# Cryptum169/another-cuda-sift

Hardware: AMD Instinct MI355X
Metric: detectAndCompute Mpix/s + 2kx2k 128-D match ms at 1/2/4/8 MI355X (higher is better)
Workload: dtype f32; 1 GPU; C2: detectAndCompute on 1920x1200 frames, 16 per step per GPU (one launch per stage for the batch), numOctaveLayers=3 (5 DoG scales/octave), numOctaves=3, upscale=false, numFeatures=5000; frames HBM-resident; frames_per_launch=16, streams_per_gpu=2, parallelism=frame-sharded x1, no data-path collective, descriptor_mode=fixed-point (default), keypoints_per_frame=4366

## Files before the change

### another-cuda-sift_amd/csrc/pyramid.hip

```cpp
#include <array>
#include <cstring>
#include <utility>

#include "sift_kernels.h"
#include "sift_math.h"

namespace sift_amd {

__device__ __forceinline__ void up_coeff(int d, int slen, int& s, float& a0, float& a1) {
    float f = (float)d * 0.5f - 0.25f;
    int si = (int)floorf(f);
    f -= (float)si;
    if (si < 0) { f = 0.f; si = 0; }
    if (si >= slen - 1) { f = 0.f; si = slen - 1; }
    s = si;
    a0 = 1.f - f;
    a1 = f;
}

__device__ __forceinline__ float dpp_left_or(float own, float v) {
    return __int_as_float(__builtin_amdgcn_update_dpp(__float_as_int(own), __float_as_int(v), 0x138, 0xf, 0xf, false));
}
__device__ __forceinline__ float dpp_right_or(float own, float v) {
    return __int_as_float(__builtin_amdgcn_update_dpp(__float_as_int(own), __float_as_int(v), 0x130, 0xf, 0xf, false));
}

template <typename T>
__global__ __launch_bounds__(256) void k_upsample2x(const T* __restrict__ src, int spitch, int W, int H,
                                                    float* __restrict__ dst, int dpitch, long sfs, long dfs) {
    src = fptr(src, blockIdx.z * sfs);
    dst = fptr(dst, blockIdx.z * dfs);
    const int per = (H + 4 * (int)gridDim.y - 1) / (4 * (int)gridDim.y);
    const int m0 = (blockIdx.y * 4 + (threadIdx.x >> 6)) * per;
    if (m0 >= H) return;
    const int mEnd = min(m0 + per, H);
    const int lane = threadIdx.x & 63, base = blockIdx.x * 256;
    const int c[2] = {base + 2 * lane, base + 128 + 2 * lane};
    const int xe = lane == 0 ? max(base - 1, 0) : min(base + 256, W - 1);
    const bool vec = sizeof(T) == 4 && (reinterpret_cast<uintptr_t>(src) & 7) == 0 && (spitch & 1) == 0;
    struct Raw {
        float v[2][2], e;
    };
    auto load = [&](int y, Raw& r) {
        const T* row = src + (size_t)min(max(y, 0), H - 1) * spitch;
#pragma unroll
        for (int h = 0; h < 2; h++) {
            if (vec && c[h] + 1 < W) {
                const float2 q = *reinterpret_cast<const float2*>(row + c[h]);
                r.v[h][0] = q.x;
                r.v[h][1] = q.y;
            } else {
                r.v[h][0] = (float)row[min(c[h], W - 1)];
                r.v[h][1] = (float)row[min(c[h] + 1, W - 1)];
            }
        }
        r.e = (float)row[xe];
    };
    auto horiz = [&](const Raw& r, float (&hh)[8]) {
        float w[2][4];
        const float a1_63 = __int_as_float(__builtin_amdgcn_readlane(__float_as_int(r.v[0][1]), 63));
        const float b0_0 = __int_as_float(__builtin_amdgcn_readlane(__float_as_int(r.v[1][0]), 0));
        w[0][0] = dpp_left_or(r.e, r.v[0][1]);
        w[0][3] = dpp_right_or(b0_0, r.v[0][0]);
        w[1][0] = dpp_left_or(a1_63, r.v[1][1]);
        w[1][3] = dpp_right_or(r.e, r.v[1][0]);
#pragma unroll
        for (int h = 0; h < 2; h++) {
            w[h][1] = r.v[h][0];
            w[h][2] = r.v[h][1];
            if (c[h] >= 1 && c[h] + 2 < W) {
                hh[4 * h] = w[h][0] * 0.25f + w[h][1] * 0.75f;
                hh[4 * h + 1] = w[h][1] * 0.75f + w[h][2] * 0.25f;
                hh[4 * h + 2] = w[h][1] * 0.25f + w[h][2] * 0.75f;
                hh[4 * h + 3] = w[h][2] * 0.75f + w[h][3] * 0.25f;
            } else {
#pragma unroll
                for (int t = 0; t < 4; t++) {
                    int sx;
                    float ax0, ax1;
                    up_coeff(min(2 * c[h] + t, 2 * W - 1), W, sx, ax0, ax1);
                    const int k0 = min(max(sx - c[h] + 1, 0), 3), k1 = min(max(min(sx + 1, W - 1) - c[h] + 1, 0), 3);
                    const float s0 = k0 == 0 ? w[h][0] : (k0 == 1 ? w[h][1] : (k0 == 2 ? w[h][2] : w[h][3]));
                    const float s1 = k1 == 0 ? w[h][0] : (k1 == 1 ? w[h][1] : (k1 == 2 ? w[h][2] : w[h][3]));
                    hh[4 * h + t] = s0 * ax0 + s1 * ax1;
                }
            }
        }
    };
    Raw rr;
    float hp[8], hc[8], hn[8];
    load(m0 - 1, rr);
    horiz(rr, hp);
    load(m0, rr);
    horiz(rr, hc);
    load(m0 + 1, rr);
    for (int m = m0; m < mEnd; m++) {
        horiz(rr, hn);
        if (m + 1 < mEnd) load(m + 2, rr);
#pragma unroll
        for (int v = 0; v < 2; v++) {
            int sy;
            float ay0, ay1;
            up_coeff(2 * m + v, H, sy, ay0, ay1);
            const bool r0c = sy == m, r1c = min(sy + 1, H - 1) == m;
            float o[8];
#pragma unroll
            for (int i = 0; i < 8; i++) o[i] = (r0c ? hc[i] : hp[i]) * ay0 + (r1c ? hc[i] : hn[i]) * ay1;
            float* d = dst + (size_t)(2 * m + v) * dpitch;
#pragma unroll
            for (int h = 0; h < 2; h++) {
                if (c[h] + 2 <= W) {
                    *reinterpret_cast<float4*>(d + 2 * c[h]) = make_float4(o[4 * h], o[4 * h + 1], o[4 * h + 2], o[4 * h + 3]);
                } else if (c[h] < W) {
                    d[2 * c[h]] = o[4 * h];
                    d[2 * c[h] + 1] = o[4 * h + 1];
                }
            }
        }
#pragma unroll
        for (int i = 0; i < 8; i++) {
            hp[i] = hc[i];
            hc[i] = hn[i];
        }
    }
}

dim3 up_grid(int W, int H, int nf) {
    const int per = nf > 1 ? 8 : 2;
    return dim3((W + 255) / 256, (H + 4 * per - 1) / (4 * per), nf);
}

void launch_upsample2x(const float* src, int spitch, int W, int H, float* dst, int dpitch, const Frames& fr, long sfs,
                       hipStream_t s) {
    hipLaunchKernelGGL(k_upsample2x<float>, up_grid(W, H, fr.nf), dim3(256), 0, s, src, spitch, W, H, dst, dpitch, sfs,
                       fr.stride);
}

void launch_upsample2x_u8(const uint8_t* src, int spitch, int W, int H, float* dst, int dpitch, const Frames& fr,
                          long sfs, hipStream_t s) {
    hipLaunchKernelGGL(k_upsample2x<uint8_t>, up_grid(W, H, fr.nf), dim3(256), 0, s, src, spitch, W, H, dst, dpitch, sfs, fr.stride);
}

typedef float f32x4 __attribute__((ext_vector_type(4)));
typedef float f32x2 __attribute__((ext_vector_type(2)));

__device__ __forceinline__ f32x2 pk_mov_hi_lo(f32x2 a, f32x2 b) {
    f32x2 r;
    __asm__("v_pk_mov_b32 %0, %1, %2 op_sel:[1,0]" : "=v"(r) : "v"(a), "v"(b));
    return r;
}
constexpr int BLUR_TW = 64;
constexpr int BLUR_TH = 64;
constexpr int kBlurBigTiles = 2048;
static_assert(BLUR_TH % 32 == 0, "blur tile height: 8-row column blocks for 4 or 8 waves");
static int blur_waves(int tiles) { return tiles >= kBlurBigTiles ? 4 : 8; }

struct BlurJob {
    const void* src;
    float* dst;
    DecOut dec;
    unsigned* range_keys;
    Counters* zero_ctr;
    int spitch, W, H, dpitch, tilesX, ntiles;
    int nf;
    long sfs, dfs;
    Taps taps;
};

constexpr bool kBlurIW16 = true;
constexpr bool kBlurX4Ld = true;
constexpr bool kBlurX4LdBig = true;
constexpr int kBlurX4LdMaxR = 24;
constexpr bool kBlurX4St = true;
constexpr bool kBlurDma = true;
template <int R>
constexpr int blur_org() {
    return kBlurX4Ld && R <= 8 ? 8 : kBlurX4Ld && kBlurX4LdBig && R <= kBlurX4LdMaxR ? (R + 3) & ~3 : R;
}
constexpr bool kBlurIW112 = false;
template <int R>
constexpr int blur_iw() {
    return kBlurIW16 && R <= 8 ? ((BLUR_TW + 2 * blur_org<R>() + 15) / 32) * 32 + 16
           : kBlurIW112 && R >= 11 && R <= 24 ? 112
                                                   : (BLUR_TW + 2 * blur_org<R>() + 3) & ~3;
}
template <int R>
constexpr int blur_lds_floats() {
    return blur_iw<R>() * (BLUR_TH + 2 * R) + 4;
}


template <int R, typename T, int NWAVES>
__device__ __forceinline__ void blur_tile(const BlurJob& J, int blk, float* __restrict__ in) {
    constexpr int BLUR_NW = NWAVES;
    constexpr int BLUR_CB = BLUR_TH / (8 * BLUR_NW);
    constexpr int IW = blur_iw<R>();
    constexpr int IH = BLUR_TH + 2 * R;
    constexpr int ORG = blur_org<R>();
    constexpr int SA = (ORG - R) & ~3, SS = (ORG - R) & 3;
    constexpr int NW = (SS + 2 * R + 4 + 3) / 4;
    static_assert(BLUR_TW - 4 + SA + 4 * NW <= IW, "row window inside the LDS row");
    const int t = xcd_tile(blk, J.ntiles * J.nf);
    const int f = t / J.ntiles, tile = t - f * J.ntiles;
    const T* __restrict__ src = fptr(static_cast<const T*>(J.src), f * J.sfs);
    float* __restrict__ dst = fptr(J.dst, f * J.dfs);
    float* __restrict__ dec_out = J.dec.p ? fptr(J.dec.p, f * J.dfs) : nullptr;
    unsigned* __restrict__ range_keys = J.range_keys ? fptr(J.range_keys, f * J.dfs) : nullptr;
    Counters* __restrict__ zero_ctr = J.zero_ctr ? fptr(J.zero_ctr, f * J.dfs) : nullptr;
    const int spitch = J.spitch, W = J.W, H = J.H, dpitch = J.dpitch;
    const Taps& taps = J.taps;
    float* const mid = in;
    const int x0 = (tile % J.tilesX) * BLUR_TW, y0 = (tile / J.tilesX) * BLUR_TH;
    const int tid = threadIdx.x, lane = tid & 63, wave = tid >> 6;
    if (zero_ctr && tile == 0 && tid < (int)(sizeof(Counters) / 4))
        reinterpret_cast<unsigned*>(zero_ctr)[tid] =
            tid == offsetof(Counters, pad[1]) / 4 ? zero_ctr->pad[1] & ~((1u << kHostReqShift) - 1) : 0u;

    {
        constexpr int RW = BLUR_TW + 2 * R;
        constexpr int RPW = (IH + BLUR_NW - 1) / BLUR_NW;
        const int wv = __builtin_amdgcn_readfirstlane(wave);
        const bool single = W > R + 1 && H > R + 1;
        auto refl = [&](int p, int len) {
            if (single) {
                p = p < 0 ? -p : (p >= len ? 2 * len - 2 - p : p);
                return min(max(p, 0), len - 1);
            }
            return reflect101(p, len);
        };
        const int gx0 = refl(x0 - R + lane, W), gx1 = refl(x0 - R + 64 + min(lane, RW - 65), W);
        constexpr int ES = (int)sizeof(T);
        const __amdgpu_buffer_rsrc_t rsrc = __builtin_amdgcn_make_buffer_rsrc(
            const_cast<T*>(src), 0, (int)min((long)spitch * H * ES, 0x7fffffffL), 0x00020000);
        const unsigned c0 = (unsigned)gx0 * ES, c1 = (unsigned)gx1 * ES;
        const int rowB = spitch * ES;
        float v0[RPW], v1[RPW];
        auto ld = [&](int i, int roff) {
            if constexpr (ES == 1) {
                v0[i] = (float)__builtin_amdgcn_raw_buffer_load_b8(rsrc, c0, roff, 0);
                v1[i] = (float)__builtin_amdgcn_raw_buffer_load_b8(rsrc, c1, roff, 0);
            } else {
                v0[i] = __builtin_bit_cast(float, __builtin_amdgcn_raw_buffer_load_b32(rsrc, c0, roff, 0));
                v1[i] = __builtin_bit_cast(float, __builtin_amdgcn_raw_buffer_load_b32(rsrc, c1, roff, 0));
            }
        };
        constexpr int QW = (BLUR_TW + 2 * ORG) / 4;
        const bool x4 = ES == 4 && ORG % 4 == 0 && ORG >= R && x0 >= ORG &&
                        x0 + BLUR_TW + ORG <= W && y0 - R >= 0 && y0 - R + IH <= H;
        if (x4) {
            static_assert(!(ES == 4 && ORG % 4 == 0) || 4 * QW <= IW, "x4 staging row inside the LDS row");
            constexpr int NQ = QW * IH, NT = 64 * BLUR_NW, QPT = (NQ + NT - 1) / NT;
            const int rb0 = (y0 - R) * spitch + x0 - ORG;
            if constexpr (kBlurDma && IW == 4 * QW) {
                const float* fsrc = reinterpret_cast<const float*>(src);
#pragma unroll
                for (int u = 0; u < QPT; u++) {
                    const int idx = tid + NT * u;
                    if (u < QPT - 1 || idx < NQ) {
                        const int row = idx / QW, qq = idx - row * QW;
                        __builtin_amdgcn_global_load_lds(
                            (const void*)(fsrc + rb0 + row * spitch + 4 * qq),
                            (__attribute__((address_space(3))) void*)(in + 4 * (NT * u + 64 * (tid >> 6))), 16, 0, 0);
                    }
                }
                __asm__ volatile("s_waitcnt vmcnt(0)" ::: "memory");
            } else {
                typedef unsigned u32x4s __attribute__((ext_vector_type(4)));
                u32x4s q4[QPT];
#pragma unroll
                for (int u = 0; u < QPT; u++) {
                    const int idx = min(tid + NT * u, NQ - 1), row = idx / QW, qq = idx - row * QW;
                    q4[u] = __builtin_amdgcn_raw_buffer_load_b128(rsrc, (unsigned)(rb0 + row * spitch + 4 * qq) * 4u, 0, 0);
                }
#pragma unroll
                for (int u = 0; u < QPT; u++) {
                    const int idx = tid + NT * u, row = idx / QW, qq = idx - row * QW;
                    if (u < QPT - 1 || idx < NQ) *reinterpret_cast<u32x4s*>(in + row * IW + 4 * qq) = q4[u];
                }
            }
        } else if (y0 - R >= 0 && y0 - R + IH <= H) {
            const int rb = __builtin_amdgcn_readfirstlane((y0 - R + wv) * rowB), rs = BLUR_NW * rowB;
#pragma unroll
            for (int i = 0; i < RPW; i++) ld(i, rb + i * rs);
        } else {
#pragma unroll
            for (int i = 0; i < RPW; i++) {
                const int ly = min(wv + BLUR_NW * i, IH - 1);
                ld(i, __builtin_amdgcn_readfirstlane(refl(y0 - R + ly, H) * rowB));
            }
        }
        float* const irow = in + wv * IW + lane + (ORG - R);
        if (!x4) {
#pragma unroll
            for (int i = 0; i < RPW; i++)
                if (i < RPW - 1 || wv + BLUR_NW * i < IH) irow[BLUR_NW * i * IW] = v0[i];
            if (lane < RW - 64) {
#pragma unroll
                for (int i = 0; i < RPW; i++)
                    if (i < RPW - 1 || wv + BLUR_NW * i < IH) irow[BLUR_NW * i * IW + 64] = v1[i];
            }
        }
    }
    __syncthreads();

    {
        const int l = lane & 31;
        const bool grpB = (l >= 4 && l < 12) || (l >= 16 && l < 20) || l >= 28;
        const int blk = grpB ? (l < 12 ? l - 4 : (l < 20 ? l - 8 : l - 16)) : (l < 4 ? l : (l < 16 ? l - 8 : l - 12));
        const int xq = blk * 4;
        for (int ly = wave * 4 + (lane >> 5) * 2 + (grpB ? 1 : 0); ly < IH; ly += 4 * BLUR_NW) {
            float win[4 * NW];
            const f32x4* p = reinterpret_cast<const f32x4*>(in + ly * IW + xq + SA);
#pragma unroll
            for (int v = 0; v < NW; v++) {
                f32x4 f = p[v];
                __asm__ volatile("" : "+v"(f));
                win[4 * v] = f[0];
                win[4 * v + 1] = f[1];
                win[4 * v + 2] = f[2];
                win[4 * v + 3] = f[3];
            }
            f32x2 pe[2 * NW], po[2 * NW - 1];
#pragma unroll
            for (int j = 0; j < 2 * NW; j++) pe[j] = (f32x2){win[2 * j], win[2 * j + 1]};
#pragma unroll
            for (int j = 0; j < 2 * NW - 1; j++) po[j] = pk_mov_hi_lo(pe[j], pe[j + 1]);
            auto pr = [&](int i) -> f32x2 {
                i += SS;
                return (i & 1) ? po[i >> 1] : pe[i >> 1];
            };
            f32x2 s2[2];
#pragma unroll
            for (int h = 0; h < 2; h++) {
                const int q = 2 * h;
                if constexpr (2 * R + 1 > 5) {
                    f32x2 a = {0.f, 0.f};
#pragma unroll
                    for (int k = 0; k <= 2 * R; k++) a = __builtin_elementwise_fma(pr(q + k), (f32x2)taps.w[k], a);
                    s2[h] = a;
                } else {
                    f32x2 a = pr(q + R) * (f32x2)taps.w[R];
#pragma unroll
                    for (int k = 1; k <= R; k++)
                        a = __builtin_elementwise_fma(pr(q + R - k) + pr(q + R + k), (f32x2)taps.w[R + k], a);
                    s2[h] = a;
                }
            }
            *reinterpret_cast<float4*>(mid + ly * IW + xq) = make_float4(s2[0][0], s2[0][1], s2[1][0], s2[1][1]);
        }
    }
    __syncthreads();

    float mx = -FLT_MAX, nmn = -FLT_MAX;
    const int gx = x0 + lane;
    const bool full = y0 + BLUR_TH <= H && x0 + BLUR_TW <= W;
    float outs[BLUR_CB][8];
#pragma unroll
    for (int cbk = 0; cbk < BLUR_CB; cbk++) {
        const int lx = lane, yb = (wave + cbk * BLUR_NW) * 8;
        const volatile __attribute__((address_space(3))) float* vmid =
            (const volatile __attribute__((address_space(3))) float*)(mid + yb * IW + lx);
        f32x2 cp[4 + 2 * R];
#pragma unroll
        for (int j = 0; j < 4 + 2 * R; j++) cp[j] = (f32x2){vmid[j * IW], vmid[(j + 4) * IW]};
        float out[8];
#pragma unroll
        for (int q = 0; q < 4; q++) {
            f32x2 a = __builtin_elementwise_fma(cp[q + R], (f32x2)taps.w[R], (f32x2){0.f, 0.f});
#pragma unroll
            for (int k = 1; k <= R; k++) a = __builtin_elementwise_fma(cp[q + R + k] + cp[q + R - k], (f32x2)taps.w[R + k], a);
            out[q] = a[0];
            out[q + 4] = a[1];
        }
        if (kBlurX4St && full) {
#pragma unroll
            for (int q = 0; q < 8; q++) outs[cbk][q] = out[q];
        } else if (full) {
            const __amdgpu_buffer_rsrc_t drs = __builtin_amdgcn_make_buffer_rsrc(
                dst, 0, (int)min((long)dpitch * H * 4, 0x7fffffffL), 0x00020000);
            const unsigned voff = (unsigned)((y0 + yb) * dpitch + gx) * 4u;
#pragma unroll
            for (int q = 0; q < 8; q++)
                __builtin_amdgcn_raw_buffer_store_b32(__builtin_bit_cast(unsigned, out[q]), drs, voff, q * dpitch * 4, 0);
        } else {
#pragma unroll
            for (int q = 0; q < 8; q++) {
                const int gy = y0 + yb + q;
                if (gy < H && gx < W) dst[(size_t)gy * dpitch + gx] = out[q];
            }
        }
        if (dec_out && !(kBlurX4St && full)) {
            const __amdgpu_buffer_rsrc_t drs = __builtin_amdgcn_make_buffer_rsrc(
                dec_out, 0, (int)min((long)J.dec.pitch * J.dec.H * 4, 0x7fffffffL), 0x00020000);
            const bool cx = (gx & 1) == 0 && (gx >> 1) < J.dec.W;
#pragma unroll
            for (int q = 0; q < 8; q += 2) {
                const int dy = (y0 + yb + q) >> 1;
                const unsigned off = cx && dy < J.dec.H ? (unsigned)(dy * J.dec.pitch + (gx >> 1)) * 4u : 0x80000000u;
                __builtin_amdgcn_raw_buffer_store_b32(__builtin_bit_cast(unsigned, out[q]), drs, off, 0, 0);
            }
        }
        if (range_keys) {
#pragma unroll
            for (int q = 0; q < 8; q++) {
                if (y0 + yb + q < H && gx < W) {
                    mx = fmaxf(mx, out[q]);
                    nmn = fmaxf(nmn, -out[q]);
                }
            }
        }
    }
    if (kBlurX4St && full) {
        __syncthreads();
#pragma unroll
        for (int cbk = 0; cbk < BLUR_CB; cbk++) {
            const int yb = (wave + cbk * BLUR_NW) * 8;
#pragma unroll
            for (int q = 0; q < 8; q++) in[(yb + q) * BLUR_TW + lane] = outs[cbk][q];
        }
        typedef unsigned u32x4t __attribute__((ext_vector_type(4)));
        const __amdgpu_buffer_rsrc_t drs =
            __builtin_amdgcn_make_buffer_rsrc(dst, 0, (int)min((long)dpitch * H * 4, 0x7fffffffL), 0x00020000);
#pragma unroll
        for (int cbk = 0; cbk < BLUR_CB; cbk++) {
            const int yb = (wave + cbk * BLUR_NW) * 8;
#pragma unroll
            for (int hh = 0; hh < 2; hh++) {
                const int row = yb + 4 * hh + (lane >> 4), c4 = 4 * (lane & 15);
                const u32x4t v = *reinterpret_cast<const u32x4t*>(in + row * BLUR_TW + c4);
                __builtin_amdgcn_raw_buffer_store_b128(v, drs, (unsigned)((y0 + row) * dpitch + x0 + c4) * 4u, 0, 0);
            }
        }
        if (dec_out) {
            const __amdgpu_buffer_rsrc_t ers = __builtin_amdgcn_make_buffer_rsrc(
                dec_out, 0, (int)min((long)J.dec.pitch * J.dec.H * 4, 0x7fffffffL), 0x00020000);
            const int r4 = (lane & 31) >> 3, c8 = 8 * (lane & 7);
#pragma unroll
            for (int it = 0; it < (BLUR_CB + 1) / 2; it++) {
                const int cbk = 2 * it + (lane >> 5);
                const int yb = (wave + min(cbk, BLUR_CB - 1) * BLUR_NW) * 8;
                const f32x4* rp = reinterpret_cast<const f32x4*>(in + (yb + 2 * r4) * BLUR_TW + c8);
                const f32x4 a = rp[0], b = rp[1];
                const u32x4t v = __builtin_bit_cast(u32x4t, (f32x4){a[0], a[2], b[0], b[2]});
                const unsigned off =
                    cbk < BLUR_CB ? (unsigned)(((y0 + yb) / 2 + r4) * J.dec.pitch + x0 / 2 + c8 / 2) * 4u : 0x80000000u;
                __builtin_amdgcn_raw_buffer_store_b128(v, ers, off, 0, 0);
            }
        }
    }
    {
        if (range_keys) {
            for (int off = 32; off > 0; off >>= 1) {
                mx = fmaxf(mx, __shfl_xor(mx, off));
                nmn = fmaxf(nmn, __shfl_xor(nmn, off));
            }
            __syncthreads();
            if (lane == 0) {
                mid[wave] = mx;
                mid[BLUR_NW + wave] = nmn;
            }
            __syncthreads();
            if (tid == 0) {
                unsigned* slot = range_keys + 2 * (tile % kRangeSlots);
                float a = mid[0], b = mid[BLUR_NW];
                for (int w = 1; w < BLUR_NW; w++) {
                    a = fmaxf(a, mid[w]);
                    b = fmaxf(b, mid[BLUR_NW + w]);
                }
                atomicMax(slot, range_key(a));
                atomicMax(slot + 1, range_key(b));
            }
        }
    }
}

template <int R, typename T, int NW>
__global__ __launch_bounds__(64 * NW) void k_blur(BlurJob J) {
    __shared__ __attribute__((aligned(16))) float in[blur_lds_floats<R>()];
    blur_tile<R, T, NW>(J, blockIdx.x, in);
}

template <int RA, int RB, int NW>
__global__ __launch_bounds__(64 * NW) void k_blur2(BlurJob A, BlurJob B) {
    constexpr int NA = blur_lds_floats<RA>(), NB = blur_lds_floats<RB>();
    __shared__ __attribute__((aligned(16))) float in[NA > NB ? NA : NB];
    const int na = A.ntiles * A.nf;
    if ((int)blockIdx.x < na)
        blur_tile<RA, float, NW>(A, blockIdx.x, in);
    else
        blur_tile<RB, float, NW>(B, blockIdx.x - na, in);
}

static BlurJob make_job(const void* src, int spitch, int W, int H, float* dst, int dpitch, const DecOut& dec,
                        const Taps& taps, unsigned* range_keys, Counters* zero_ctr, const Frames& fr, long sfs) {
    BlurJob j;
    j.nf = fr.nf;
    j.sfs = sfs;
    j.dfs = fr.stride;
    j.src = src;
    j.dst = dst;
    j.dec = dec;
    j.range_keys = range_keys;
    j.zero_ctr = zero_ctr;
    j.spitch = spitch;
    j.W = W;
    j.H = H;
    j.dpitch = dpitch;
    j.tilesX = (W + BLUR_TW - 1) / BLUR_TW;
    j.ntiles = j.tilesX * ((H + BLUR_TH - 1) / BLUR_TH);
    j.taps = taps;
    return j;
}

using BlurLaunch = void (*)(const BlurJob&, hipStream_t);

template <int R>
void blur_launch_r(const BlurJob& j, hipStream_t s) {
    const int tiles = j.ntiles * j.nf;
    if (blur_waves(tiles) == 4)
        hipLaunchKernelGGL((k_blur<R, float, 4>), dim3(tiles), dim3(256), 0, s, j);
    else
        hipLaunchKernelGGL((k_blur<R, float, 8>), dim3(tiles), dim3(512), 0, s, j);
}

template <int... Rs>
constexpr std::array<BlurLaunch, sizeof...(Rs)> blur_table(std::integer_sequence<int, Rs...>) {
    return {&blur_launch_r<Rs + 1>...};
}
static const std::array<BlurLaunch, kMaxTaps / 2> kBlurTable = blur_table(std::make_integer_sequence<int, kMaxTaps / 2>{});

template <int RA, int RB>
void blur2_launch(const BlurJob& a, const BlurJob& b, hipStream_t s) {
    const int tiles = a.ntiles * a.nf + b.ntiles * b.nf;
    if (blur_waves(tiles) == 4)
        hipLaunchKernelGGL((k_blur2<RA, RB, 4>), dim3(tiles), dim3(256), 0, s, a, b);
    else
        hipLaunchKernelGGL((k_blur2<RA, RB, 8>), dim3(tiles), dim3(512), 0, s, a, b);
}
bool launch_blur_pair_jobs(const BlurJob& a, const BlurJob& b, hipStream_t s) {
    const int ra = a.taps.n >> 1, rb = b.taps.n >> 1;
#define SIFT_PAIR(X, Y)                      \
    if (ra == X && rb == Y) {                \
        blur2_launch<X, Y>(a, b, s);         \
        return true;                         \
    }                                        \
    if (ra == Y && rb == X) {                \
        blur2_launch<X, Y>(b, a, s);         \
        return true;                         \
    }
    SIFT_PAIR(6, 5)
    SIFT_PAIR(8, 5)
    SIFT_PAIR(8, 6)
    SIFT_PAIR(10, 5)
    SIFT_PAIR(10, 6)
    SIFT_PAIR(10, 8)
    SIFT_PAIR(13, 5)
    SIFT_PAIR(13, 6)
    SIFT_PAIR(13, 8)
    SIFT_PAIR(13, 10)
#undef SIFT_PAIR
    return false;
}

bool launch_blur_pair(const BlurDesc& a, const BlurDesc& b, const Frames& fr, hipStream_t s) {
    return launch_blur_pair_jobs(make_job(a.src, a.spitch, a.W, a.H, a.dst, a.dpitch, a.dec, *a.taps,
                                          nullptr, nullptr, fr, fr.stride),
                                 make_job(b.src, b.spitch, b.W, b.H, b.dst, b.dpitch, b.dec, *b.taps,
                                          nullptr, nullptr, fr, fr.stride),
                                 s);
}

bool launch_blur_u8(const uint8_t* src, int spitch, int W, int H, float* dst, int dpitch, const Taps& taps,
                    const Frames& fr, long sfs, hipStream_t s, unsigned* range_keys, Counters* zero_ctr) {
    const BlurJob j = make_job(src, spitch, W, H, dst, dpitch, DecOut{}, taps, range_keys, zero_ctr, fr, sfs);
    const int tiles = j.ntiles * j.nf;
    const bool big = blur_waves(tiles) == 4;
    switch (taps.n >> 1) {
        case 5:
            if (big) hipLaunchKernelGGL((k_blur<5, uint8_t, 4>), dim3(tiles), dim3(256), 0, s, j);
            else hipLaunchKernelGGL((k_blur<5, uint8_t, 8>), dim3(tiles), dim3(512), 0, s, j);
            return true;
        case 6:
            if (big) hipLaunchKernelGGL((k_blur<6, uint8_t, 4>), dim3(tiles), dim3(256), 0, s, j);
            else hipLaunchKernelGGL((k_blur<6, uint8_t, 8>), dim3(tiles), dim3(512), 0, s, j);
            return true;
        default: return false;
    }
}

__global__ __launch_bounds__(256) void k_u8_to_f32(const uint8_t* __restrict__ src, int spitch, int W, int H,
                                                   float* __restrict__ dst, int dpitch, long sfs, long dfs) {
    src = fptr(src, blockIdx.z * sfs);
    dst = fptr(dst, blockIdx.z * dfs);
    const int x = blockIdx.x * 256 + threadIdx.x, y = blockIdx.y;
    if (x < W) dst[(size_t)y * dpitch + x] = (float)src[(size_t)y * spitch + x];
}

void launch_u8_to_f32(const uint8_t* src, int spitch, int W, int H, float* dst, int dpitch, const Frames& fr,
                      long sfs, hipStream_t s) {
    hipLaunchKernelGGL(k_u8_to_f32, dim3((W + 255) / 256, H, fr.nf), dim3(256), 0, s, src, spitch, W, H, dst, dpitch,
                       sfs, fr.stride);
}

template <int R>
const void* blur_fn(int nw) {
    return nw == 4 ? reinterpret_cast<const void*>(&k_blur<R, float, 4>)
                   : reinterpret_cast<const void*>(&k_blur<R, float, 8>);
}
template <int... Rs>
constexpr std::array<const void* (*)(int), sizeof...(Rs)> blur_fn_table(std::integer_sequence<int, Rs...>) {
    return {&blur_fn<Rs + 1>...};
}
static const std::array<const void* (*)(int), kMaxTaps / 2> kBlurFnTable =
    blur_fn_table(std::make_integer_sequence<int, kMaxTaps / 2>{});
static_assert(sizeof(BlurJob) <= sizeof(HeadNode::args), "head node argument storage");

void head_blur_node(HeadNode& h, const float* src, int spitch, int W, int H, float* dst, int dpitch, const Taps& taps,
                    const Frames& fr, long sfs, unsigned* range_keys, Counters* zero_ctr) {
    const BlurJob j = make_job(src, spitch, W, H, dst, dpitch, DecOut{}, taps, range_keys, zero_ctr, fr, sfs);
    const int tiles = j.ntiles * j.nf, nw = blur_waves(tiles);
    std::memcpy(h.args, &j, sizeof j);
    h.argv[0] = h.args;
    h.p = hipKernelNodeParams{};
    h.p.func = const_cast<void*>(kBlurFnTable[(taps.n >> 1) - 1](nw));
    h.p.gridDim = dim3(tiles);
    h.p.blockDim = dim3(64 * nw);
    h.p.sharedMemBytes = 0;
    h.p.kernelParams = h.argv;
    h.p.extra = nullptr;
}

void head_upsample_node(HeadNode& h, const float* src, int spitch, int W, int H, float* dst, int dpitch,
                        const Frames& fr, long sfs) {
    unsigned char* a = h.args;
    auto put = [&](int i, const void* v, size_t n) {
        std::memcpy(a + 16 * i, v, n);
        h.argv[i] = a + 16 * i;
    };
    put(0, &src, sizeof src);
    put(1, &spitch, sizeof spitch);
    put(2, &W, sizeof W);
    put(3, &H, sizeof H);
    put(4, &dst, sizeof dst);
    put(5, &dpitch, sizeof dpitch);
    put(6, &sfs, sizeof sfs);
    put(7, &fr.stride, sizeof fr.stride);
    h.p = hipKernelNodeParams{};
    h.p.func = reinterpret_cast<void*>(&k_upsample2x<float>);
    h.p.gridDim = up_grid(W, H, fr.nf);
    h.p.blockDim = dim3(256);
    h.p.sharedMemBytes = 0;
    h.p.kernelParams = h.argv;
    h.p.extra = nullptr;
}

void launch_blur(const float* src, int spitch, int W, int H, float* dst, int dpitch, const DecOut& dec,
                 const Taps& taps, const Frames& fr, long sfs, hipStream_t s, unsigned* range_keys,
                 Counters* zero_ctr) {
    const int r = taps.n >> 1;
    kBlurTable[r - 1](make_job(src, spitch, W, H, dst, dpitch, dec, taps, range_keys, zero_ctr, fr, sfs), s);
}

constexpr int kTailThreads = 1024;
constexpr int kTailRun = 4;
constexpr int kTailRmax = 16;
constexpr int kTailMaxDim = 512;

__host__ __device__ __forceinline__ int tail_pitch(int W) { return W | 1; }

__device__ __forceinline__ void gstore(float* p, size_t i, float v) {
    ((__attribute__((address_space(1))) float*)p)[i] = v;
}
__device__ __forceinline__ float gload(const float* p, size_t i) {
    return ((const __attribute__((address_space(1))) float*)p)[i];
}

template <int RP>
__device__ __forceinline__ void tail_row_pass(const float* __restrict__ A, float* __restrict__ B, int W, int H, int P,
                                              bool small, const float* __restrict__ wp, const int* __restrict__ xo) {
    constexpr int NWIN = kTailRun + 2 * RP;
    const int nrx = (W + kTailRun - 1) / kTailRun, nruns = nrx * H;
    for (int r = threadIdx.x; r < nruns; r += kTailThreads) {
        const int y = r % H, xb = (r / H) * kTailRun;
        const float* row = A + y * P;
        float win[NWIN];
        if (xb - RP >= 0 && xb + kTailRun - 1 + RP < W) {
#pragma unroll
            for (int k = 0; k < NWIN; k++) win[k] = row[xb - RP + k];
        } else {
            int ix[NWIN];
#pragma unroll
            for (int k = 0; k < NWIN; k++) ix[k] = xo[xb + k];
#pragma unroll
            for (int k = 0; k < NWIN; k++) win[k] = row[ix[k]];
        }
        float s[kTailRun];
        if (!small) {
#pragma unroll
            for (int q = 0; q < kTailRun; q++) s[q] = 0.f;
#pragma unroll
            for (int k = 0; k <= 2 * RP; k++) {
                const float wk = wp[k];
#pragma unroll
                for (int q = 0; q < kTailRun; q++) s[q] = __fmaf_rn(win[q + k], wk, s[q]);
            }
        } else {
            const float wc = wp[RP];
#pragma unroll
            for (int q = 0; q < kTailRun; q++) s[q] = win[q + RP] * wc;
#pragma unroll
            for (int k = 1; k <= 2 && k <= RP; k++) {
                const float wk = wp[RP + k];
#pragma unroll
                for (int q = 0; q < kTailRun; q++) s[q] = __fmaf_rn(win[q + RP - k] + win[q + RP + k], wk, s[q]);
            }
        }
#pragma unroll
        for (int q = 0; q < kTailRun; q++)
            if (xb + q < W) B[y * P + xb + q] = s[q];
    }
}

template <int RP>
__device__ __forceinline__ void tail_col_pass(const float* __restrict__ B, float* __restrict__ A, int W, int H, int P,
                                              const float* __restrict__ wp, const int* __restrict__ yo,
                                              float* __restrict__ gdst, int gpitch, bool dec, float* __restrict__ N,
                                              int NP, float* __restrict__ gnext, int gnpitch) {
    constexpr int NWIN = kTailRun + 2 * RP;
    const int nry = (H + kTailRun - 1) / kTailRun, nruns = nry * W;
    for (int r = threadIdx.x; r < nruns; r += kTailThreads) {
        const int x = r % W, yb = (r / W) * kTailRun;
        float win[NWIN];
        if (yb - RP >= 0 && yb + kTailRun - 1 + RP < H) {
#pragma unroll
            for (int k = 0; k < NWIN; k++) win[k] = B[(yb - RP + k) * P + x];
        } else {
            int iy[NWIN];
#pragma unroll
            for (int k = 0; k < NWIN; k++) iy[k] = yo[yb + k];
#pragma unroll
            for (int k = 0; k < NWIN; k++) win[k] = B[iy[k] * P + x];
        }
        float s[kTailRun];
        const float wc = wp[RP];
#pragma unroll
        for (int q = 0; q < kTailRun; q++) s[q] = __fmaf_rn(win[q + RP], wc, 0.f);
#pragma unroll
        for (int k = 1; k <= RP; k++) {
            const float wk = wp[RP + k];
#pragma unroll
            for (int q = 0; q < kTailRun; q++) s[q] = __fmaf_rn(win[q + RP + k] + win[q + RP - k], wk, s[q]);
        }
#pragma unroll
        for (int q = 0; q < kTailRun; q++) {
            const int y = yb + q;
            if (y < H) {
                A[y * P + x] = s[q];
#if !defined(SIFT_TAIL_DIAG) || SIFT_TAIL_DIAG != 4
                gstore(gdst, (size_t)y * gpitch + x, s[q]);
#endif
                if (dec && !((x | y) & 1) && (x >> 1) < (W >> 1) && (y >> 1) < (H >> 1)) {
                    N[(y >> 1) * NP + (x >> 1)] = s[q];
                    gstore(gnext, (size_t)(y >> 1) * gnpitch + (x >> 1), s[q]);
                }
            }
        }
    }
}

template <int RP>
__device__ __forceinline__ void tail_octaves(const TailDesc& T, float* lds, const float (*wall)[2 * kTailRmax + 1],
                                             int* xo, int* yo, long foff) {
    int aOff = 0, nOff = T.regionX;
    const int bOff = T.regionX + T.regionY;
    for (int o = T.o0; o < T.nOct; o++) {
        const OctGeom& g = T.oct[o];
        const OctGeom& gn = T.oct[o + 1 < T.nOct ? o + 1 : o];
        float* base = fptr(g.base, foff);
        const int P = tail_pitch(g.W);
        lds_barrier();
        const int t = threadIdx.x;
        if (t < g.W + 2 * RP + kTailRun) xo[t] = reflect101(min(t - RP, g.W - 1 + RP), g.W);
        if (t < g.H + 2 * RP + kTailRun) yo[t] = reflect101(min(t - RP, g.H - 1 + RP), g.H);
        for (int i = 1; i < T.L + 3; i++) {
#if defined(SIFT_TAIL_DIAG) && SIFT_TAIL_DIAG == 5
            if (threadIdx.x == 0) {
                const unsigned long long t0 = __builtin_amdgcn_s_memtime();
                unsigned* st = reinterpret_cast<unsigned*>(fptr(T.oct[0].base, foff));
                const int slot = (o - T.o0) * (T.L + 2) + (i - 1);
                st[2 * slot] = (unsigned)t0;
                st[2 * slot + 1] = (unsigned)(t0 >> 32);
            }
#endif
            const bool small = T.taps[i].n <= 5, dec = o + 1 < T.nOct && i == T.L;
            const float* wp = wall[i];
            lds_barrier();
#if !defined(SIFT_TAIL_DIAG) || SIFT_TAIL_DIAG != 1
            tail_row_pass<RP>(lds + aOff, lds + bOff, g.W, g.H, P, small, wp, xo);
#endif
            lds_barrier();
#if !defined(SIFT_TAIL_DIAG) || SIFT_TAIL_DIAG != 2
            tail_col_pass<RP>(lds + bOff, lds + aOff, g.W, g.H, P, wp, yo, base + (size_t)i * g.planeStride, g.pitch,
                              dec, lds + nOff, tail_pitch(gn.W), dec ? fptr(gn.base, foff) : base, gn.pitch);
#endif
        }
        const int tt = aOff;
        aOff = nOff;
        nOff = tt;
    }
}

__global__ __launch_bounds__(kTailThreads) void k_blur_tail(TailDesc T, long fs) {
    extern __shared__ __attribute__((aligned(16))) float lds[];
    __shared__ float wall[kTailMaxPlanes][2 * kTailRmax + 1];
    __shared__ int xo[kTailMaxDim + 2 * kTailRmax + kTailRun], yo[kTailMaxDim + 2 * kTailRmax + kTailRun];
    const long foff = (long)blockIdx.x * fs;
    const int RP = T.rpad;
    {
        for (int t = threadIdx.x; t < kTailMaxPlanes * (2 * kTailRmax + 1); t += kTailThreads) {
            const int i = t / (2 * kTailRmax + 1), k = t - i * (2 * kTailRmax + 1);
// ... 453 lines not shown
```

### another-cuda-sift_amd/csrc/sift_kernels.h

```cpp
#pragma once
#include <hip/hip_runtime.h>
#include <stdint.h>

#include <string>

namespace sift_amd {

constexpr int kMaxOctaves = 16;
constexpr int kMaxTaps = 63;
constexpr int kMaxBatch = 64;

struct Frames {
    int nf;
    long stride;
};
template <class T>
__host__ __device__ __forceinline__ T* fptr(T* p, long off) {
    return reinterpret_cast<T*>(reinterpret_cast<uintptr_t>(p) + off);
}

struct Taps {
    float w[64];
    int n;
};

struct OctGeom {
    float* base;
    long planeStride;
    int W, H, pitch;
    int rowBase;
    long bitBase;
};

struct PyrDesc {
    OctGeom oct[kMaxOctaves];
    int nOct;
    int L;
    int firstOctave;
};

struct RefKpt {
    float x, y, size, response;
    int octave;
    int o, layer, rc;
};

struct OriKpt {
    float x, y, size, angle, response;
    int octave;
    int bucket, sub;
};

struct Counters {
    unsigned cand;
    unsigned refined;
    unsigned oriented;
    unsigned final_n;
    unsigned overflow;
    unsigned thr_bits;
    unsigned pad[2];
};

constexpr unsigned kHoleBucket = 0xffffffffu;

void launch_upsample2x(const float* src, int spitch, int W, int H, float* dst, int dpitch, const Frames& fr, long sfs,
                       hipStream_t s);
constexpr int kRangeSlots = 256;
struct DecOut {
    float* p = nullptr;
    int pitch = 0, W = 0, H = 0;
};
void launch_blur(const float* src, int spitch, int W, int H, float* dst, int dpitch, const DecOut& dec,
                 const Taps& taps, const Frames& fr, long sfs, hipStream_t s, unsigned* range_keys = nullptr,
                 Counters* zero_ctr = nullptr);
struct HeadNode {
    hipKernelNodeParams p;
    alignas(16) unsigned char args[512];
    void* argv[8];
};
void head_blur_node(HeadNode& h, const float* src, int spitch, int W, int H, float* dst, int dpitch, const Taps& taps,
                    const Frames& fr, long sfs, unsigned* range_keys, Counters* zero_ctr);
void head_upsample_node(HeadNode& h, const float* src, int spitch, int W, int H, float* dst, int dpitch,
                        const Frames& fr, long sfs);
struct BlurDesc {
    const float* src;
    int spitch, W, H;
    float* dst;
    int dpitch;
    DecOut dec;
    const Taps* taps;
};
bool launch_blur_pair(const BlurDesc& a, const BlurDesc& b, const Frames& fr, hipStream_t s);
constexpr int kTailLdsFloats = 32768;
constexpr int kTailMaxPlanes = 9;
struct TailDesc {
    OctGeom oct[kMaxOctaves];
    Taps taps[kTailMaxPlanes];
    int o0, nOct, L, regionX, regionY, rpad;
};
int tail_first_octave(const PyrDesc& pyr, const Taps* taps, int L);
hipError_t tail_init();
void launch_blur_tail(const PyrDesc& pyr, const Taps* taps, int L, int o0, const Frames& fr, hipStream_t s);
bool launch_blur_u8(const uint8_t* src, int spitch, int W, int H, float* dst, int dpitch, const Taps& taps,
                    const Frames& fr, long sfs, hipStream_t s, unsigned* range_keys, Counters* zero_ctr);
void launch_u8_to_f32(const uint8_t* src, int spitch, int W, int H, float* dst, int dpitch, const Frames& fr,
                      long sfs, hipStream_t s);
void launch_upsample2x_u8(const uint8_t* src, int spitch, int W, int H, float* dst, int dpitch, const Frames& fr,
                          long sfs, hipStream_t s);
bool launch_extrema_all(const PyrDesc& pyr, float threshold, uint2* cand, Counters* ctr, unsigned cap,
                        const Frames& fr, hipStream_t s);
void launch_extrema(const PyrDesc& pyr, int o, float threshold, uint2* cand, Counters* ctr, unsigned cap,
                    const Frames& fr, hipStream_t s);

struct KeypointParams {
    float contrastThreshold, edgeThreshold, sigma;
    int numFeatures;
    unsigned capRefined, capOriented, capFinal;
    int numBuckets;
    int oriRmax, descRmax;
    int descNrec;
    int descExact;
};
struct MaskArg {
    const uint8_t* p = nullptr;
    int stride = 0, W = 0, H = 0;
    long fstride = 0;
};
__device__ __forceinline__ bool mask_ok(const MaskArg& m, unsigned frame, float x, float y) {
    if (!m.p) return true;
    const int ix = min(max((int)__fadd_rn(x, 0.5f), 0), m.W - 1);
    const int iy = min(max((int)__fadd_rn(y, 0.5f), 0), m.H - 1);
    return m.p[(size_t)frame * (size_t)m.fstride + (size_t)iy * (size_t)m.stride + (size_t)ix] != 0;
}

void launch_refine(const PyrDesc& pyr, const uint2* cand, unsigned capCand, Counters* ctr, uint32_t* bitmap,
                   RefKpt* out, const KeypointParams& kp, const Frames& fr, hipStream_t s);
void launch_orientation(const PyrDesc& pyr, const RefKpt* in, Counters* ctr, OriKpt* out, uint32_t* bitmap,
                        const KeypointParams& kp, const Frames& fr, hipStream_t s, const MaskArg& mask = MaskArg{});
void launch_select(const OriKpt* kpts, Counters* ctr, unsigned* zero_range, const KeypointParams& kp, const Frames& fr,
                   hipStream_t s);
constexpr int kOrderMaxBuckets = 16384;

constexpr int kLptSegs = kMaxOctaves * 8;
struct JobOrder {
    int valid;
    int segStart[kLptSegs];
    int jobBase[kLptSegs];
};

bool launch_order(const PyrDesc& pyr, const OriKpt* kpts, Counters* ctr, unsigned* zero_range, unsigned* bcount, unsigned* boff, int* slot,
                  int* order, JobOrder* jord, const KeypointParams& kp, const Frames& fr, hipStream_t s,
                  const MaskArg& mask = MaskArg{});
void launch_bucket_count(const OriKpt* kpts, const Counters* ctr, unsigned* bcount, int* slot,
                         const KeypointParams& kp, const Frames& fr, hipStream_t s, const MaskArg& mask = MaskArg{});
void launch_bucket_scan(unsigned* bcount, unsigned* boff, Counters* ctr, const KeypointParams& kp, const Frames& fr,
                        hipStream_t s);
void launch_bucket_scatter(const OriKpt* kpts, const Counters* ctr, const unsigned* boff, const int* slot,
                           int* order, const KeypointParams& kp, const Frames& fr, hipStream_t s);
constexpr int kDescMaxRows = 128;
struct DescJob {
    const float* img;
    float cos_t, sin_t;
    float angle;
    float hist_width;
    int ptx, pty;
    int rows, cols, pitch;
    int radius;
    int out;
    int pad[3];
};

static_assert(sizeof(DescJob) == 64, "DescJob is one 64-byte scalar load");

void launch_rank_final(const PyrDesc& pyr, const OriKpt* kpts, const unsigned* bcount, const unsigned* boff,
                       const int* order, const Counters* ctr, const JobOrder* jord, DescJob* jobs, float* kpts3, float* feats4,
                       const KeypointParams& kp, const Frames& fr, hipStream_t s);

struct ProvidedKpt {
    float x, y, size, angle, response;
    int octave;
};
static_assert(sizeof(ProvidedKpt) == 24, "ProvidedKpt is sift_hip_keypoint");
constexpr unsigned kFlagBadKeypoint = 16u;

__host__ __device__ inline bool provided_kpt_valid(const ProvidedKpt& k, int firstOctave, int nOct, int L, int W, int H) {
    int o = k.octave & 255;
    o = o < 128 ? o : (-128 | o);
    const int layer = (k.octave >> 8) & 255;
    const float big = 3.402823466e+38f;
    return o >= firstOctave && o <= firstOctave + nOct - 1 && layer <= L + 2 &&
           (k.x < 0 ? -k.x : k.x) <= big && (k.y < 0 ? -k.y : k.y) <= big && k.size <= big && k.size > 0.f &&
           k.angle >= 0.f && k.angle <= 360.f && k.x >= -(float)W && k.x <= 2.f * (float)W && k.y >= -(float)H &&
           k.y <= 2.f * (float)H;
}

void launch_provided_jobs(const PyrDesc& pyr, const ProvidedKpt* kpts, int n, int W, int H, Counters* ctr,
                          unsigned* zero_range, DescJob* jobs, float* kpts3, float* feats4, hipStream_t s);
constexpr int kStageWg = 64;
constexpr int kGroupCopyWg = 512;
void launch_copy_rows(const void* src, size_t spitch, void* dst, size_t dpitch, size_t rowB, int rows, int wgs,
                      hipStream_t s, unsigned* flag = nullptr, unsigned flag_val = 0);
void launch_bucket_rank(const PyrDesc& pyr, const OriKpt* kpts, unsigned* bcount, const unsigned* boff,
                        const int* order, const Counters* ctr, DescJob* jobs, float* kpts3, float* feats4,
                        const KeypointParams& kp, const Frames& fr, hipStream_t s);
struct Sidecar {
    int8_t* codes;
    int* keys;
};
constexpr int kHostReqShift = 16;
struct HostOut {
    char* const* tab;
    const float* k3;
    const float* f4;
    unsigned cap;
};
void launch_descriptor(const DescJob* jobs, const Counters* ctr, const unsigned* range_keys, uint16_t* desc,
                       Sidecar side, Counters* host_ctr, HostOut host, const KeypointParams& kp, const Frames& fr,
                       hipStream_t s);

__device__ __forceinline__ unsigned range_key(float f) {
    const unsigned u = __float_as_uint(f);
    return u & 0x80000000u ? ~u : u | 0x80000000u;
}
__device__ __forceinline__ float decode_range_key(unsigned u) {
    return __uint_as_float(u & 0x80000000u ? u & 0x7fffffffu : ~u);
}

void set_last_error(const std::string& msg);

void upload_exp_table(const float* tab64);
void upload_desc_exp_table(const float* tab64);

}
```

Baseline: 30140 Mpix/s.

## Add streaming column-strip blur kernel with register ring for radius-9 blurs

Adds a new Gaussian blur path in which each wave walks down a vertical strip of columns, doing the horizontal pass through a per-wave LDS row and keeping the last 2R+1 horizontal results in a register ring for the vertical pass. This replaces the 2D tile kernel, and its halo re-reads between tiles, for large batched blurs. Default selection enables it only for radius 9 without a decimated output. Segment overlap still re-reads 2R rows per segment, and register pressure from the ring may limit occupancy.

```diff
diff --git a/another-cuda-sift_amd/csrc/pyramid.hip b/another-cuda-sift_amd/csrc/pyramid.hip
--- a/another-cuda-sift_amd/csrc/pyramid.hip
+++ b/another-cuda-sift_amd/csrc/pyramid.hip
@@ -2,6 +2,7 @@
 #include <cstring>
 #include <utility>
 
+#include "sift_blur_plan.h"
 #include "sift_kernels.h"
 #include "sift_math.h"
 
@@ -164,6 +165,7 @@
     int spitch, W, H, dpitch, tilesX, ntiles;
     int nf;
     long sfs, dfs;
+    int sStrips, sSegRows, sNseg, sWaves, sBlocks;
     Taps taps;
 };
 
@@ -474,10 +476,194 @@
     }
 }
 
-template <int R, typename T, int NW>
+template <int R, int CPL>
+struct StreamGeom {
+    static constexpr int RING = 2 * R + 1;
+    static constexpr int SW = 64 * CPL;
+    static constexpr int ORG = (R + CPL - 1) / CPL * CPL;
+    static constexpr int SS = ORG - R;
+    static constexpr int NV = (SS + 2 * R + CPL + CPL - 1) / CPL;
+    static constexpr int LW = CPL * (63 + NV);
+    static constexpr int AHEAD = 3;
+    static constexpr int XTRA = RING % AHEAD, NSLOT = AHEAD + XTRA;
+    static constexpr int slot(int u) { return u < RING - XTRA ? u % AHEAD : AHEAD + (u - (RING - XTRA)); }
+    static_assert(ORG + SW + R <= LW, "right halo inside the LDS row");
+    static_assert(AHEAD <= RING && 2 * R <= 64, "prologue and halo lanes");
+};
+template <int R>
+constexpr int blur_stream_lds_floats() {
+    return kStreamWavesPerWg * StreamGeom<R, blur_stream_cpl(R)>::LW;
+}
+
+template <int R, int CPL, bool FULL>
+__device__ __forceinline__ void blur_stream_wave_rows(const BlurJob& J, const BlurStreamWave& sw, float* __restrict__ row) {
+    using G = StreamGeom<R, CPL>;
+    constexpr int RING = G::RING, SW = G::SW, ORG = G::ORG, SS = G::SS, NV = G::NV, H2 = CPL / 2;
+    constexpr bool fullStrip = FULL;
+    typedef float fvec __attribute__((ext_vector_type(CPL)));
+    typedef unsigned uvec __attribute__((ext_vector_type(CPL)));
+    const int lane = threadIdx.x & 63;
+    const float* __restrict__ src = fptr(static_cast<const float*>(J.src), sw.frame * J.sfs);
+    float* __restrict__ dst = fptr(J.dst, sw.frame * J.dfs);
+    const int W = J.W, H = J.H;
+    const Taps& taps = J.taps;
+    const int xs = sw.strip * SW, c0 = xs + CPL * lane;
+
+    const __amdgpu_buffer_rsrc_t srs = __builtin_amdgcn_make_buffer_rsrc(
+        const_cast<float*>(src), 0, (int)min((long)J.spitch * H * 4, 0x7fffffffL), 0x00020000);
+    const __amdgpu_buffer_rsrc_t drs =
+        __builtin_amdgcn_make_buffer_rsrc(dst, 0, (int)min((long)J.dpitch * H * 4, 0x7fffffffL), 0x00020000);
+    auto colB = [&](int c) { return (unsigned)min(max(stream_reflect(c, W), 0), W - 1) * 4u; };
+    unsigned offm[CPL], offd[CPL];
+#pragma unroll
+    for (int c = 0; c < CPL; c++) {
+        offm[c] = colB(c0 + c);
+        offd[c] = c0 + c < W ? (unsigned)(c0 + c) * 4u : 0x80000000u;
+    }
+    const int hl = min(lane, 2 * R - 1);
+    const unsigned offh = colB(hl < R ? xs - R + hl : xs + SW + hl - R);
+    float* const hrow = row + (hl < R ? SS + hl : ORG + SW + hl - R);
+    const int y0 = sw.y0, total = sw.y1 - sw.y0 + 2 * R;
+
+    struct Raw {
+        fvec v;
+        float e;
+    };
+    auto load = [&](int j, Raw& r) {
+        const int soff = stream_input_row(y0, R, min(j, total - 1), H) * J.spitch * 4;
+        if constexpr (fullStrip) {
+            if constexpr (CPL == 4)
+                r.v = __builtin_bit_cast(fvec, __builtin_amdgcn_raw_buffer_load_b128(srs, offm[0], soff, 0));
+            else
+                r.v = __builtin_bit_cast(fvec, __builtin_amdgcn_raw_buffer_load_b64(srs, offm[0], soff, 0));
+        } else {
+#pragma unroll
+            for (int c = 0; c < CPL; c++)
+                r.v[c] = __builtin_bit_cast(float, __builtin_amdgcn_raw_buffer_load_b32(srs, offm[c], soff, 0));
+        }
+        r.e = __builtin_bit_cast(float, __builtin_amdgcn_raw_buffer_load_b32(srs, offh, soff, 0));
+    };
+    const bool hasDec = J.dec.p != nullptr;
+    __amdgpu_buffer_rsrc_t ers = drs;
+    unsigned offe[H2];
+#pragma unroll
+    for (int h = 0; h < H2; h++) offe[h] = 0x80000000u;
+    if (hasDec) {
+        ers = __builtin_amdgcn_make_buffer_rsrc(fptr(J.dec.p, sw.frame * J.dfs), 0,
+                                                (int)min((long)J.dec.pitch * J.dec.H * 4, 0x7fffffffL), 0x00020000);
+#pragma unroll
+        for (int h = 0; h < H2; h++)
+            if (c0 + 2 * h < W && c0 / 2 + h < J.dec.W) offe[h] = (unsigned)(c0 / 2 + h) * 4u;
+    }
+
+    Raw raw[G::NSLOT];
+    f32x2 ring[RING][H2];
+#pragma unroll
+    for (int u = 0; u < G::AHEAD; u++) load(u, raw[G::slot(u)]);
+    for (int jb = 0; jb < total; jb += RING) {
+#pragma unroll
+        for (int u = 0; u < RING; u++) {
+            const int j = jb + u;
+            *reinterpret_cast<fvec*>(row + ORG + CPL * lane) = raw[G::slot(u)].v;
+            if (lane < 2 * R) *hrow = raw[G::slot(u)].e;
+            load(j + G::AHEAD, raw[G::slot((u + G::AHEAD) % RING)]);
+            __builtin_amdgcn_fence(__ATOMIC_ACQ_REL, "wavefront");
+            __builtin_amdgcn_wave_barrier();
+            float win[CPL * NV];
+            const fvec* p = reinterpret_cast<const fvec*>(row + CPL * lane);
+#pragma unroll
+            for (int v = 0; v < NV; v++) {
+                fvec f = p[v];
+                __asm__ volatile("" : "+v"(f));
+#pragma unroll
+                for (int c = 0; c < CPL; c++) win[CPL * v + c] = f[c];
+            }
+            __builtin_amdgcn_fence(__ATOMIC_ACQ_REL, "wavefront");
+            __builtin_amdgcn_wave_barrier();
+            constexpr int NP = CPL * NV / 2;
+            f32x2 pe[NP], po[NP - 1];
+#pragma unroll
+            for (int i = 0; i < NP; i++) pe[i] = (f32x2){win[2 * i], win[2 * i + 1]};
+#pragma unroll
+            for (int i = 0; i < NP - 1; i++) po[i] = pk_mov_hi_lo(pe[i], pe[i + 1]);
+            auto pr = [&](int i) -> f32x2 {
+                i += SS;
+                return (i & 1) ? po[i >> 1] : pe[i >> 1];
+            };
+            f32x2 acc[H2];
+#pragma unroll
+            for (int h = 0; h < H2; h++) acc[h] = (f32x2){0.f, 0.f};
+#pragma unroll
+            for (int k = 0; k <= 2 * R; k++)
+#pragma unroll
+                for (int h = 0; h < H2; h++) acc[h] = __builtin_elementwise_fma(pr(2 * h + k), (f32x2)taps.w[k], acc[h]);
+#pragma unroll
+            for (int h = 0; h < H2; h++) ring[u][h] = acc[h];
+            if (j >= 2 * R && j < total) {
+                const int y = y0 + j - 2 * R;
+                const int ctr = (u + R + 1) % RING;
+                f32x2 o[H2];
+#pragma unroll
+                for (int h = 0; h < H2; h++)
+                    o[h] = __builtin_elementwise_fma(ring[ctr][h], (f32x2)taps.w[R], (f32x2){0.f, 0.f});
+#pragma unroll
+                for (int k = 1; k <= R; k++)
+#pragma unroll
+                    for (int h = 0; h < H2; h++)
+                        o[h] = __builtin_elementwise_fma(ring[(ctr + k) % RING][h] + ring[(ctr + RING - k) % RING][h],
+                                                         (f32x2)taps.w[R + k], o[h]);
+                const int doff = y * J.dpitch * 4;
+                if constexpr (fullStrip) {
+                    if constexpr (CPL == 4)
+                        __builtin_amdgcn_raw_buffer_store_b128(
+                            __builtin_bit_cast(uvec, __builtin_shufflevector(o[0], o[H2 - 1], 0, 1, 2, 3)), drs, offd[0],
+                            doff, 0);
+                    else
+                        __builtin_amdgcn_raw_buffer_store_b64(__builtin_bit_cast(uvec, o[0]), drs, offd[0], doff, 0);
+                } else {
+#pragma unroll
+                    for (int h = 0; h < H2; h++) {
+                        const float lo = o[h][0], hi = o[h][1];
+                        __builtin_amdgcn_raw_buffer_store_b32(__builtin_bit_cast(unsigned, lo), drs, offd[2 * h], doff, 0);
+                        __builtin_amdgcn_raw_buffer_store_b32(__builtin_bit_cast(unsigned, hi), drs, offd[2 * h + 1], doff, 0);
+                    }
+                }
+                if (hasDec && (y & 1) == 0 && (y >> 1) < J.dec.H) {
+                    const int eoff = (y >> 1) * J.dec.pitch * 4;
+#pragma unroll
+                    for (int h = 0; h < H2; h++) {
+                        const float lo = o[h][0];
+                        __builtin_amdgcn_raw_buffer_store_b32(__builtin_bit_cast(unsigned, lo), ers, offe[h], eoff, 0);
+                    }
+                }
+            }
+        }
+    }
+}
+
+template <int R, int CPL>
+__device__ __forceinline__ void blur_stream(const BlurJob& J, int blk, float* __restrict__ lds) {
+    using G = StreamGeom<R, CPL>;
+    const int wave = __builtin_amdgcn_readfirstlane(threadIdx.x >> 6);
+    const int wid = xcd_tile(blk, J.sBlocks) * kStreamWavesPerWg + wave;
+    if (wid >= J.sWaves) return;
+    const BlurStreamWave sw = blur_stream_wave(wid, J.sStrips, J.sSegRows, J.sNseg, J.H);
+    float* const row = lds + wave * G::LW;
+    if (sw.strip * G::SW + G::SW <= J.W)
+        blur_stream_wave_rows<R, CPL, true>(J, sw, row);
+    else
+        blur_stream_wave_rows<R, CPL, false>(J, sw, row);
+}
+
+template <int R, typename T, int NW, bool STREAM = false>
 __global__ __launch_bounds__(64 * NW) void k_blur(BlurJob J) {
-    __shared__ __attribute__((aligned(16))) float in[blur_lds_floats<R>()];
-    blur_tile<R, T, NW>(J, blockIdx.x, in);
+    if constexpr (STREAM) {
+        __shared__ __attribute__((aligned(16))) float rows[blur_stream_lds_floats<R>()];
+        blur_stream<R, blur_stream_cpl(R)>(J, blockIdx.x, rows);
+    } else {
+        __shared__ __attribute__((aligned(16))) float in[blur_lds_floats<R>()];
+        blur_tile<R, T, NW>(J, blockIdx.x, in);
+    }
 }
 
 template <int RA, int RB, int NW>
@@ -509,13 +695,41 @@
     j.tilesX = (W + BLUR_TW - 1) / BLUR_TW;
     j.ntiles = j.tilesX * ((H + BLUR_TH - 1) / BLUR_TH);
     j.taps = taps;
+    j.sStrips = j.sSegRows = j.sNseg = j.sWaves = j.sBlocks = 0;
     return j;
 }
 
+static int g_streamMode = -1, g_streamSegRows = 0;
+void blur_stream_override(int mode, int segRows) {
+    g_streamMode = mode;
+    g_streamSegRows = segRows;
+}
+static bool plan_stream(BlurJob& j) {
+    if (g_streamMode == 0 || j.range_keys || j.zero_ctr) return false;
+    if (g_streamMode < 0 && !blur_stream_wins(j.taps.n >> 1, j.dec.p != nullptr)) return false;
+    const auto al = [](const void* p) { return (reinterpret_cast<uintptr_t>(p) & 15) == 0; };
+    if (!al(j.src) || !al(j.dst) || (j.spitch & 3) || (j.dpitch & 3) || (j.sfs & 15) || (j.dfs & 15)) return false;
+    const BlurStreamPlan p = blur_stream_plan(j.W, j.H, j.taps.n >> 1, j.nf, g_streamSegRows);
+    if (!p.stream) return false;
+    j.sStrips = p.strips;
+    j.sSegRows = p.segRows;
+    j.sNseg = p.nseg;
+    j.sWaves = p.waves;
+    j.sBlocks = p.blocks;
+    return true;
+}
+
 using BlurLaunch = void (*)(const BlurJob&, hipStream_t);
 
 template <int R>
-void blur_launch_r(const BlurJob& j, hipStream_t s) {
+void blur_launch_r(const BlurJob& job, hipStream_t s) {
+    BlurJob j = job;
+    if constexpr (R >= kStreamRmin && R <= kStreamRmax) {
+        if (plan_stream(j)) {
+            hipLaunchKernelGGL((k_blur<R, float, 4, true>), dim3(j.sBlocks), dim3(256), 0, s, j);
+            return;
+        }
+    }
     const int tiles = j.ntiles * j.nf;
     if (blur_waves(tiles) == 4)
         hipLaunchKernelGGL((k_blur<R, float, 4>), dim3(tiles), dim3(256), 0, s, j);
diff --git a/another-cuda-sift_amd/csrc/sift_blur_plan.h b/another-cuda-sift_amd/csrc/sift_blur_plan.h
--- /dev/null
+++ b/another-cuda-sift_amd/csrc/sift_blur_plan.h
@@ -0,0 +1,80 @@
+#pragma once
+
+namespace sift_amd {
+
+constexpr int kStreamRmin = 5, kStreamRmax = 14;
+constexpr int kStreamBigTiles = 2048;
+constexpr int kStreamWavesPerWg = 4;
+constexpr int kStreamCus = 256;
+
+constexpr int blur_stream_cpl(int R) { return R <= kStreamRmax ? 4 : 2; }
+
+constexpr bool blur_stream_wins(int R, bool dec) { return R == 9 && !dec; }
+
+struct BlurStreamPlan {
+    int stream;
+    int cpl;
+    int strips;
+    int segRows;
+    int nseg;
+    int waves;
+    int blocks;
+};
+
+#if defined(__HIPCC__) || defined(__CUDACC__)
+#define SIFT_PLAN_HD __host__ __device__
+#else
+#define SIFT_PLAN_HD
+#endif
+
+SIFT_PLAN_HD inline int stream_reflect(int p, int len) {
+    return p < 0 ? -p : (p >= len ? 2 * len - 2 - p : p);
+}
+SIFT_PLAN_HD inline int stream_input_row(int y0, int R, int j, int H) { return stream_reflect(y0 - R + j, H); }
+
+constexpr int blur_stream_min_w(int cpl) { return 64 * cpl; }
+constexpr int blur_stream_min_h(int R) { return 2 * R + 1; }
+
+inline BlurStreamPlan blur_stream_plan(int W, int H, int R, int nf, int segRowsWanted = 0) {
+    BlurStreamPlan p{};
+    if (R < kStreamRmin || R > kStreamRmax || nf < 1) return p;
+    const int cpl = blur_stream_cpl(R);
+    if (W < blur_stream_min_w(cpl) || H < blur_stream_min_h(R)) return p;
+    const long tiles = (long)((W + 63) / 64) * ((H + 63) / 64) * nf;
+    if (tiles < kStreamBigTiles) return p;
+    const int strips = (W + 64 * cpl - 1) / (64 * cpl);
+    int segRows = segRowsWanted;
+    if (segRows <= 0) {
+        const long perSeg = (long)nf * strips;
+        long nseg = (2L * kStreamCus * kStreamWavesPerWg) / perSeg;
+        if (nseg < 1) nseg = 1;
+        segRows = (int)((H + nseg - 1) / nseg);
+        if (segRows < 4 * R) segRows = 4 * R;
+        const int ring = 2 * R + 1;
+        segRows = (segRows - 1 + ring - 1) / ring * ring + 1;
+    }
+    if (segRows > H) segRows = H;
+    p.stream = 1;
+    p.cpl = cpl;
+    p.strips = strips;
+    p.segRows = segRows;
+    p.nseg = (H + segRows - 1) / segRows;
+    p.waves = nf * p.nseg * strips;
+    p.blocks = (p.waves + kStreamWavesPerWg - 1) / kStreamWavesPerWg;
+    return p;
+}
+
+struct BlurStreamWave {
+    int frame, strip, y0, y1;
+};
+SIFT_PLAN_HD inline BlurStreamWave blur_stream_wave(int w, int strips, int segRows, int nseg, int H) {
+    const int strip = w % strips, r = w / strips, seg = r % nseg;
+    BlurStreamWave o;
+    o.frame = r / nseg;
+    o.y0 = seg * segRows;
+    o.y1 = o.y0 + segRows < H ? o.y0 + segRows : H;
+    o.strip = strip;
+    return o;
+}
+
+}
diff --git a/another-cuda-sift_amd/csrc/sift_kernels.h b/another-cuda-sift_amd/csrc/sift_kernels.h
--- a/another-cuda-sift_amd/csrc/sift_kernels.h
+++ b/another-cuda-sift_amd/csrc/sift_kernels.h
@@ -73,6 +73,7 @@
 void launch_blur(const float* src, int spitch, int W, int H, float* dst, int dpitch, const DecOut& dec,
                  const Taps& taps, const Frames& fr, long sfs, hipStream_t s, unsigned* range_keys = nullptr,
                  Counters* zero_ctr = nullptr);
+void blur_stream_override(int mode, int segRows);
 struct HeadNode {
     hipKernelNodeParams p;
     alignas(16) unsigned char args[512];
```

Result: faster. 30640 Mpix/s (median of 5 runs) (+1.7%).
